# joaobuibergen/roms-trunk-mgh

Hardware: AMD Instinct MI355X
Metric: simulated-days/wall-sec (higher is better)
Workload: dtype f64; 1 GPU; BENCHMARK3 2048x256x30 NT=2 nonlinear 3-D step incl. 59 step2d calls, U3/C4 tracer advection, analytic atmospheric forcing, bulk fluxes + KPP + diagnostics every step; tiling=1x1, halo_transport=none, rccl_ranks=0, graph_exchanges=1, ndtfast=20, finite=True

## Files before the change

### include/roms_hip.h

```cpp
#ifndef ROMS_HIP_H
#define ROMS_HIP_H

#ifdef __cplusplus
extern "C" {
#endif

enum roms_kind {
  K_2D = 0, K_2D_T2, K_2D_T3, K_2D_NT,
  K_3DR, K_3DW, K_3DR_T2, K_3DW_T2, K_3DW_NAT, K_4DT, K_3DR_NT, K_3DW_T3
};

enum roms_field_id {
#define ROMS_FIELD(name, kind, owner) FID_##name,
#include "roms_fields.def"
#undef ROMS_FIELD
  FID_COUNT
};

typedef struct roms_fields {
#define ROMS_FIELD(name, kind, owner) double *name;
#include "roms_fields.def"
#undef ROMS_FIELD
} roms_fields_t;

// ... 129 lines not shown
int roms_hip_get_diagnostic(int dia_id, int itrc, int accumulated, double *host, long n_doubles);
int roms_hip_dia_index(int dia_id, int hdif, int rotated);
int roms_hip_set_floats(int Nfloats, const int *Ftype, const double *Tinfo, const double *Fz0,
                        const double *xcoord, const double *ycoord);
int roms_hip_floats_put(const double *track, long n_track, const int *bounded, long n_bounded);
int roms_hip_floats_get(double *track, long n_track, int *bounded, long n_bounded);
int roms_hip_step_floats(const roms_step_idx_t *s, double time, const int nfl[5]);
int roms_hip_set_tides(int NTC, int MTC, const double *Tperiod, const double *SSH_Tamp, const double *SSH_Tphase,
                       const double *UV_Tangle, const double *UV_Tphase, const double *UV_Tmajor, const double *UV_Tminor,
                       const double *angler, double tide_start, int ramp_tides, double dstart,
                       int add_fsobc, const double *zeta_base, int add_m2obc, const double *ubar_base,
                       const double *vbar_base);
int roms_hip_tides(double time);
int roms_hip_wvelocity(const roms_step_idx_t *s);
int roms_hip_diag(const roms_step_idx_t *s, double *out12);

int roms_hip_step2d_loop(roms_step_idx_t *s, int *indx1);

int roms_hip_graph_exchanges(int on);
int roms_hip_graph_exchanges_state(void);

int roms_hip_exchange(int field_id, int level);

typedef struct { int peer; int tag; long count; double *buf; } roms_halo_msg_t;
typedef int (*roms_halo_relay_fn)(void *user, int nsend, const roms_halo_msg_t *send,
                                  int nrecv, const roms_halo_msg_t *recv);
int roms_hip_set_halo_relay(roms_halo_relay_fn fn, void *user);
int roms_hip_halo_plan(const roms_bounds_t *b, int rank, int *out);

int roms_hip_timing_enable(int on);
// ... 11 lines not shown
```

### roms_trunk_mgh_amd/abi.py

```python
import ctypes as C
import keyword
import os
import re

ROOT = os.path.dirname(os.path.dirname(os.path.abspath(__file__)))
INCLUDE_DIR = os.path.join(ROOT, "include")


def _read(name):
    with open(os.path.join(INCLUDE_DIR, name)) as fh:
        return re.sub(r"/\*.*?\*/", "", fh.read(), flags=re.S)


def _constants():
    txt = _read("roms_hip.h")
    out = {n: int(v) for n, v in re.findall(r"^#define\s+(\w+)\s+(\d+)\s*$", txt, flags=re.M)}
    for body in re.findall(r"\benum\s+\w+\s*\{([^{}#]*)\}", txt):
        nxt = 0
        for item in body.split(","):
            name, _, val = (x.strip() for x in item.partition("="))
            out[name] = nxt = int(val) if val else nxt
            nxt += 1
    return out

# ... 7 lines not shown

ADV = {"C2": 0, "C4": 1, "A4": 2, "U3": 3, "SU3": 4, "SPLINES": 5,
       "MPDATA": 6, "HSIMT": 7}
GLS_STAB = {"GALPERIN": 0, "KANTHA_CLAYSON": 1, "CANUTO_A": 2, "CANUTO_B": 3}
PGF = {"DJ_GRADPS": 0, "STANDARD": 1, "WJ_GRADP": 2, "PJ_GRADP": 3}
LBC_PERIODIC, LBC_CLOSED, LBC_GRADIENT, LBC_CLAMPED, LBC_CHAPMAN_IMPLICIT, LBC_FLATHER, LBC_RADIATION = range(7)
LBC = {"Per": 0, "Clo": 1, "Gra": 2, "Cla": 3, "Cha": 4, "Fla": 5, "Rad": 6, "RadNud": 7, "Che": 8, "Shc": 9, "Red": 10}
UV_HADV = {"U3": 0, "C2": 1, "C4": 2}
UV_VADV = {"C4W": 0, "C2": 1, "C4": 2, "SPLINES": 3}
UV_ADV_PAIRS = [("U3", "C4W"), ("U3", "SPLINES"), ("C2", "C2"), ("C2", "SPLINES"), ("C4", "C4"), ("C4", "SPLINES")]


def uv_adv(h="U3", v="C4W"):
    return 1 | (UV_HADV.get(h, h) << 4) | (UV_VADV.get(v, v) << 8)


LBV = {"zeta": 0, "ubar": 1, "vbar": 2, "u": 3, "v": 4, "t": 5}
LBS = {"west": 0, "east": 1, "south": 2, "north": 3}


FIELDS = re.findall(r"\bROMS_FIELD\(\s*(\w+)\s*,\s*(\w+)\s*,\s*(\w+)\s*\)", _read("roms_fields.def"))
FIELD_ID = {n: i for i, (n, _, _) in enumerate(FIELDS)}
FIELD_KIND = {n: k for n, k, _ in FIELDS}


def trailing_shape(kind, N, NT, NAT):
    return {
        "K_2D": (), "K_2D_T2": (2,), "K_2D_T3": (3,), "K_2D_NT": (NT,),
        "K_3DR": (N,), "K_3DW": (N + 1,), "K_3DR_T2": (N, 2),
        "K_3DW_T2": (N + 1, 2), "K_3DW_NAT": (N + 1, NAT), "K_4DT": (N, 3, NT), "K_3DR_NT": (N, NT),
# ... 71 lines not shown
```

### roms_trunk_mgh_amd/csrc/capi.hip

```cpp
#include "roms_dev.h"
#include <algorithm>
#include <map>
#include <vector>

RomsCtx g_ctx;

static const int k_field_kind[FID_COUNT] = {
#define ROMS_FIELD(name, kind, owner) kind,
#include "roms_fields.def"
#undef ROMS_FIELD
};
static const char *k_field_name[FID_COUNT] = {
#define ROMS_FIELD(name, kind, owner) #name,
#include "roms_fields.def"
#undef ROMS_FIELD
};

int roms_fail(const char *where, const char *what)
{
  g_ctx.last_error = std::string(where) + ": " + what;
  return 8;
}

long roms_field_count(int kind, const roms_bounds_t &b)
// ... 23 lines not shown
  if (!g_ctx.timing) return;
  if (hipEventCreate(&e0) != hipSuccess || hipEventCreate(&e1) != hipSuccess) { e0 = e1 = nullptr; return; }
  (void)hipEventRecord(e0, g_ctx.stream);
}
ScopedTimer::~ScopedTimer()
{
  if (!e0) return;
  float ms = 0.f;
  if (hipEventRecord(e1, g_ctx.stream) == hipSuccess && hipEventSynchronize(e1) == hipSuccess &&
      hipEventElapsedTime(&ms, e0, e1) == hipSuccess)
    g_last_ms[name] = ms;
  (void)hipEventDestroy(e0);
  (void)hipEventDestroy(e1);
}

extern "C" int roms_hip_timing_enable(int on) { g_ctx.timing = on != 0; return 0; }
extern "C" double roms_hip_timing_last_ms(const char *entry)
{
  auto it = g_last_ms.find(entry);
  return it == g_last_ms.end() ? -1.0 : it->second;
}

__global__ void __launch_bounds__(256) k_calib_stream(const double *__restrict__ src, double *__restrict__ dst, long n)
{
  const long e = (long)blockIdx.x * 256 + threadIdx.x;
  if (e < n) dst[e] = src[e];
}
int roms_entry_check(const char *where);
namespace { void sources_release(); void clima_release(); void avg_release(); }
extern "C" int roms_hip_calib_stream(long n)
// ... 718 lines not shown
```

### roms_trunk_mgh_amd/csrc/k_diag.hip

```cpp
#include "roms_dev.h"

int roms_entry_check(const char *name);

namespace {

__global__ void __launch_bounds__(BLK_X *BLK_Y)
k_wvelocity(const RomsDev *__restrict__ c, int ninp)
{
  DEV_PROLOGUE(c)
  const Blk XB = xcd_block();
  const int i = b.Istr + XB.x * BLK_X + threadIdx.x;
  const int j = b.Jstr + XB.y * BLK_Y + threadIdx.y;
  if (i > b.Iend || j > b.Jend) return;
  const long a = I2(i, j);
  const gcd_t u = (gcd_t)(c->F.u + (long)(ninp - 1) * n3r), v = (gcd_t)(c->F.v + (long)(ninp - 1) * n3r);
  const gcd_t z_r = (gcd_t)c->F.z_r, z_w = (gcd_t)c->F.z_w, W = (gcd_t)c->F.W;
  const gd_t wvel = (gd_t)c->F.wvel;
  const gcd_t pm = (gcd_t)c->F.pm, pn = (gcd_t)c->F.pn;
  const double pmw = pm[a - 1] + pm[a], pme = pm[a] + pm[a + 1];
  const double pns = pn[a - ni] + pn[a], pnn = pn[a] + pn[a + ni];
  const double pmn = pm[a] * pn[a];
  auto vert_at = [&](int k) {
    const long q = a + (long)(k - 1) * nij;
    const double zr0 = z_r[q];
// ... 17 lines not shown
  }
  double vm = v1, v0 = v2, vp = v3;
  for (int k = 2; k <= N - 2; k++) {
    const double vq = vert_at(k + 2);
    wvel[w3i(k)] = pmn * (W[w3i(k)] + wrk * (z_w[w3i(k)] - zw0)) + cff4 * (v0 + vp) - cff5 * (vm + vq);
    vm = v0; v0 = vp; vp = vq;
  }
  {
    const long qN = a + (long)(N - 1) * nij;
    const double slope = (zwN - z_r[qN]) / (z_r[qN] - z_r[qN - nij]);
    wvel[w3i(N)] = pmn * wrk * (zwN - zw0) + cff1 * (vp + slope * (vp - v0)) + cff2 * vp - cff3 * v0;
    wvel[w3i(N - 1)] = pmn * (W[w3i(N - 1)] + wrk * (z_w[w3i(N - 1)] - zw0)) + cff1 * vp + cff2 * v0 - cff3 * vm;
  }
}

struct DiagScratch { double *ke, *pe, *C, *Cu, *Cv, *Cw, *Ck, *spd, *rho, *vol; };

__global__ void __launch_bounds__(BLK_X *BLK_Y)
k_diag_col(const RomsDev *__restrict__ c, int idia, DiagScratch w)
{
  DEV_PROLOGUE(c)
  const roms_params_t &p = c->p;
  const Blk XB = xcd_block();
  const int i = b.Istr + XB.x * BLK_X + threadIdx.x;
  const int j = b.Jstr + XB.y * BLK_Y + threadIdx.y;
  if (i > b.Iend || j > b.Jend) return;
  const long a = I2(i, j);
  const gcd_t u = (gcd_t)(c->F.u + (long)(idia - 1) * n3r), v = (gcd_t)(c->F.v + (long)(idia - 1) * n3r);
  const gcd_t Hz = (gcd_t)c->F.Hz, z_r = (gcd_t)c->F.z_r, z_w = (gcd_t)c->F.z_w, rho = (gcd_t)c->F.rho;
  const gcd_t wvel = (gcd_t)c->F.wvel;
  const double zwN = z_w[a + (long)N * nij], zw0 = z_w[a];
  const double pm = GF(pm)[a], pn = GF(pn)[a], dt = p.dt;
  double ke = 0.0, pe = 0.5 * p.g * zwN * zwN;
  const double cff = p.g / p.rho0;
  double mC = 0.0, mCu = 0.0, mCv = 0.0, mCw = 0.0, mspd = 0.0, mrho = -1.0E+37;
  int mk = 0;
  double wv_up = wvel[a + (long)N * nij];
  for (int k = N; k >= 1; k--) {
    const long q = a + (long)(k - 1) * nij;
    const double u0 = u[q], u1 = u[q + 1], v0 = v[q], v1 = v[q + ni], hz = Hz[q], rh = rho[q];
    const double wv_dn = wvel[q];
    const double u2v2 = u0 * u0 + u1 * u1 + v0 * v0 + v1 * v1;
    ke = ke + hz * 0.25 * u2v2;
    pe = pe + cff * hz * (rh + 1000.0) * (z_r[q] - zw0);
    const double Cu = 0.5 * fabs(u0 + u1) * dt * pm;
    const double Cv = 0.5 * fabs(v0 + v1) * dt * pn;
    const double Cw = 0.5 * fabs(wv_dn + wv_up) * dt / hz;
    const double C = Cu + Cv + Cw;
    if (C > mC) { mC = C; mCu = Cu; mCv = Cv; mCw = Cw; mk = k; }
    mspd = fmax(mspd, sqrt(0.5 * u2v2));
    mrho = fmax(mrho, rh);
    wv_up = wv_dn;
  }
  const double om = GF(omn)[a];
  w.vol[a] = om * (zwN - zw0);
  ke = om * ke;
  pe = om * pe;
  w.ke[a] = ke; w.pe[a] = pe; w.C[a] = mC; w.Cu[a] = mCu; w.Cv[a] = mCv; w.Cw[a] = mCw; w.Ck[a] = (double)mk;
  w.spd[a] = mspd; w.rho[a] = mrho;
}

enum { R_VOL = 0, R_PE, R_KE, R_C, R_CU, R_CV, R_CW, R_CJ, R_CK, R_SPD, R_RHO, R_COUNT };

#define DIAG_UNR 16
__global__ void __launch_bounds__(64)
k_diag_rows(const RomsDev *__restrict__ c, DiagScratch w, double *__restrict__ R)
{
  DEV_PROLOGUE(c)
  const int i = b.Istr + blockIdx.x * blockDim.x + threadIdx.x;
  if (i > b.Iend) return;
  const int nI = b.Iend - b.Istr + 1, o = i - b.Istr;
  const gcd_t gvol = (gcd_t)w.vol, gpe = (gcd_t)w.pe, gke = (gcd_t)w.ke, gC = (gcd_t)w.C, gspd = (gcd_t)w.spd,
              grho = (gcd_t)w.rho;
  double vol = 0.0, pe = 0.0, ke = 0.0, mC = 0.0, mCu = 0.0, mCv = 0.0, mCw = 0.0, mspd = 0.0, mrho = -1.0E+37;
// ... 136 lines not shown
  const roms_bounds_t &b = g_ctx.b;
  if (b.N < 3) return roms_fail("roms_hip_wvelocity", "needs N >= 3");
  halo_batch_begin();
  halo_exchange2d(GT_U, g_ctx.dev[FID_DU_avg1]);
  halo_exchange2d(GT_V, g_ctx.dev[FID_DV_avg1]);
  if ((rc = halo_batch_end())) return rc;
  {
    ScopedTimer tm("wvelocity");
    hipLaunchKernelGGL(k_wvelocity, grid2d(b.Iend - b.Istr + 1, b.Jend - b.Jstr + 1), block2d(), 0, g_ctx.stream,
                       g_ctx.devc, s->nstp);
    KERNEL_CHECK("k_wvelocity");
  }
  return bc_w3d(g_ctx.dev[FID_wvel]);
}

extern "C" int roms_hip_diag(const roms_step_idx_t *s, double *out12)
{
  int rc = roms_entry_check("roms_hip_diag");
  if (rc) return rc;
  if (!out12) return roms_fail("roms_hip_diag", "null output");
  const roms_bounds_t &b = g_ctx.b;
  const int nI = b.Iend - b.Istr + 1, nJ = b.Jend - b.Jstr + 1;
  if (!g_diag_dev) HIP_TRY(hipMalloc(&g_diag_dev, 12 * sizeof(double)));
  if (g_diag_rows_n < (long)R_COUNT * nI) {
    if (g_diag_rows) HIP_TRY(hipFree(g_diag_rows));
    g_diag_rows = nullptr;
    HIP_TRY(hipMalloc(&g_diag_rows, sizeof(double) * R_COUNT * nI));
    g_diag_rows_n = (long)R_COUNT * nI;
  }
  double **ws = g_ctx.hostc.ws2;
  DiagScratch w{ws[8], ws[9], ws[10], ws[11], ws[12], ws[13], ws[14], ws[15], ws[16], ws[17]};
  {
    ScopedTimer tm("diag");
    hipLaunchKernelGGL(k_diag_col, grid2d(nI, nJ), block2d(), 0, g_ctx.stream, g_ctx.devc, s->nstp, w);
    KERNEL_CHECK("k_diag_col");
    hipLaunchKernelGGL(k_diag_rows, dim3((nI + 63) / 64), dim3(64), 0, g_ctx.stream, g_ctx.devc, w, g_diag_rows);
    KERNEL_CHECK("k_diag_rows");
    hipLaunchKernelGGL(k_diag_final, dim3(1), dim3(256), 0, g_ctx.stream, g_ctx.devc, (const double *)g_diag_rows,
                       g_diag_dev);
    KERNEL_CHECK("k_diag_final");
  }
  HIP_TRY(hipMemcpyAsync(out12, g_diag_dev, 12 * sizeof(double), hipMemcpyDeviceToHost, g_ctx.stream));
  HIP_TRY(hipStreamSynchronize(g_ctx.stream));
  return 0;
}
```

### roms_trunk_mgh_amd/csrc/k_rho_eos.hip

```cpp
#include "roms_dev.h"
#include "roms_eoscoef.h"

int roms_entry_check(const char *name);

namespace {

struct EosPt {
  double den1, bulk0, bulk1, bulk2, bulk, den;
  double Dden1DS, Dden1DT, DbulkDS, DbulkDT;
};

template <bool DERIV>
__device__ __forceinline__ EosPt eos_point(double tt, double ts, double Tp)
{
  EosPt o;
  const double Tt = (-2.0 > tt) ? -2.0 : tt;
  const double Ts = (0.0 > ts) ? 0.0 : ts;
  const double sqrtTs = sqrt(Ts);
  const double Tpr10 = 0.1 * Tp;
  const double C0 = EOS_Q00 + Tt * (EOS_Q01 + Tt * (EOS_Q02 + Tt * (EOS_Q03 + Tt * (EOS_Q04 + Tt * EOS_Q05))));
  const double C1 = EOS_U00 + Tt * (EOS_U01 + Tt * (EOS_U02 + Tt * (EOS_U03 + Tt * EOS_U04)));
  const double C2 = EOS_V00 + Tt * (EOS_V01 + Tt * EOS_V02);
  o.den1 = C0 + Ts * (C1 + sqrtTs * C2 + Ts * EOS_W00);
  const double C3 = EOS_A00 + Tt * (EOS_A01 + Tt * (EOS_A02 + Tt * (EOS_A03 + Tt * EOS_A04)));
// ... 17 lines not shown
    o.Dden1DS = C1 + 1.5 * C2 * sqrtTs + 2.0 * EOS_W00 * Ts;
    o.Dden1DT = d0 + Ts * (d1 + sqrtTs * d2);
    const double d3 = EOS_A01 + Tt * (2.0 * EOS_A02 + Tt * (3.0 * EOS_A03 + Tt * 4.0 * EOS_A04));
    const double d4 = EOS_B01 + Tt * (2.0 * EOS_B02 + Tt * 3.0 * EOS_B03);
    const double d5 = EOS_D01 + Tt * 2.0 * EOS_D02;
    const double d6 = EOS_E01 + Tt * (2.0 * EOS_E02 + Tt * 3.0 * EOS_E03);
    const double d7 = EOS_F01 + Tt * 2.0 * EOS_F02;
    const double d8 = EOS_G02 + Tt * 2.0 * EOS_G03;
    const double d9 = EOS_H01 + Tt * 2.0 * EOS_H02;
    o.DbulkDS = C4 + sqrtTs * 1.5 * C5 - Tp * (C7 + sqrtTs * 1.5 * EOS_G00 - Tp * C9);
    o.DbulkDT = d3 + Ts * (d4 + sqrtTs * d5) - Tp * (d6 + Ts * d7 - Tp * (d8 + Ts * d9));
  }
  return o;
}

__global__ void __launch_bounds__(BLK_X *BLK_Y)
k_rho_eos_nonlin(const RomsDev *__restrict__ c, int nrhs)
{
  DEV_PROLOGUE(c)
  const Blk XB = xcd_block();
  const int i = b.IstrT + XB.x * BLK_X + threadIdx.x;
  const int j = b.JstrT + XB.y * BLK_Y + threadIdx.y;
  if (i > b.IendT || j > b.JendT) return;
  const long c0 = I2(i, j);
  const gcd_t T = (gcd_t)(c->F.t + (long)(nrhs - 1) * n3r);
  const gcd_t S = (gcd_t)(c->F.t + ((long)(nrhs - 1) + 3L) * n3r);
  const bool salt = c->p.salinity != 0 && b.NT >= 2;
  const gcd_t z_r = (gcd_t)(c->F.z_r);
  const gcd_t z_w = (gcd_t)(c->F.z_w);
  const gcd_t Hz = (gcd_t)(c->F.Hz);
  const double g = c->p.g;
  double rhoA = 0.0, rhoS = 0.0;
  EosPt up{};
  double zr_up = 0.0;
  const bool masking = c->p.masking != 0;
  const double rm = masking ? GF(rmask)[c0] : 1.0;
  for (int k = N; k >= 1; k--) {
    const long ck = c0 + (long)(k - 1) * nij;
    const double zr = z_r[ck], hz = Hz[ck];
    const double tt = T[ck], ts = salt ? S[ck] : 0.0;
    EosPt e;
    if (k == N) {
      e = eos_point<true>(tt, ts, zr);
      if (masking) e.den = e.den * rm;
      const double Tpr10 = 0.1 * zr;
      const double cff = e.bulk + Tpr10;
      const double cff1 = Tpr10 * e.den1;
      const double cff2 = e.bulk * cff;
      const double wrk = (e.den + 1000.0) * cff * cff;
      const double Tcof = -(e.DbulkDT * cff1 + e.Dden1DT * cff2);
      const double Scof = (e.DbulkDS * cff1 + e.Dden1DS * cff2);
// ... 9 lines not shown
      if (masking) e.den = e.den * rm;
      const double cf1 = e.den * hz;
      rhoS = rhoS + hz * (rhoA + 0.5 * cf1);
      rhoA = rhoA + cf1;
      const double zw = z_w[c0 + (long)k * nij];
      const double bulk_up = up.bulk0 - zw * (up.bulk1 - up.bulk2 * zw);
      const double bulk_dn = e.bulk0 - zw * (e.bulk1 - e.bulk2 * zw);
      const double c1 = 1.0 / (bulk_up + 0.1 * zw);
      const double c2 = 1.0 / (bulk_dn + 0.1 * zw);
      const double den_up = c1 * (up.den1 * bulk_up);
      const double den_dn = c2 * (e.den1 * bulk_dn);
      GF(bvf)[c0 + (long)k * nij] = -g * (den_up - den_dn) / (0.5 * (den_up + den_dn) * (zr_up - zr));
    }
    GF(rho)[ck] = e.den;
    GF(pden)[ck] = masking ? (e.den1 - 1000.0) * rm : e.den1 - 1000.0;
    up = e;
    zr_up = zr;
  }
  GF(bvf)[c0] = 0.0;
  const double cff2 = 1.0 / c->p.rho0;
  const double cff1 = 1.0 / (z_w[c0 + (long)N * nij] - z_w[c0]);
  GF(rhoA)[c0] = cff2 * cff1 * rhoA;
  GF(rhoS)[c0] = 2.0 * cff1 * cff1 * cff2 * rhoS;
}

__global__ void __launch_bounds__(BLK_X *BLK_Y)
k_rho_eos_lin(const RomsDev *__restrict__ c, int nrhs)
{
  DEV_PROLOGUE(c)
  const Blk XB = xcd_block();
  const int i = b.IstrT + XB.x * BLK_X + threadIdx.x;
  const int j = b.JstrT + XB.y * BLK_Y + threadIdx.y;
  if (i > b.IendT || j > b.JendT) return;
  const long c0 = I2(i, j);
  const gcd_t T = (gcd_t)(c->F.t + (long)(nrhs - 1) * n3r);
  const gcd_t S = (gcd_t)(c->F.t + ((long)(nrhs - 1) + 3L) * n3r);
  const bool salt = c->p.salinity != 0 && b.NT >= 2;
  const double R0 = c->p.R0, T0 = c->p.T0, S0 = c->p.S0, Tcoef = c->p.Tcoef, Scoef = c->p.Scoef;
// ... 11 lines not shown
    if (k == N) { rhoS = 0.5 * cf1 * hz; rhoA = cf1; }
    else { rhoS = rhoS + hz * (rhoA + 0.5 * cf1); rhoA = rhoA + cf1; }
  }
  const double cff2 = 1.0 / c->p.rho0;
  const double cff1 = 1.0 / (GF(z_w)[c0 + (long)N * nij] - GF(z_w)[c0]);
  GF(rhoA)[c0] = cff2 * cff1 * rhoA;
  GF(rhoS)[c0] = 2.0 * cff1 * cff1 * cff2 * rhoS;
}

}

extern "C" int roms_hip_rho_eos(const roms_step_idx_t *s)
{
  int rc = roms_entry_check("roms_hip_rho_eos");
  if (rc) return rc;
  ScopedTimer tm("rho_eos");
  const roms_bounds_t &b = g_ctx.b;
  dim3 grid = grid2d(b.IendT - b.IstrT + 1, b.JendT - b.JstrT + 1);
  if (g_ctx.p.nonlin_eos)
    hipLaunchKernelGGL(k_rho_eos_nonlin, grid, block2d(), 0, g_ctx.stream, g_ctx.devc, s->nrhs);
  else
    hipLaunchKernelGGL(k_rho_eos_lin, grid, block2d(), 0, g_ctx.stream, g_ctx.devc, s->nrhs);
  KERNEL_CHECK("k_rho_eos");
  halo_batch_begin();
  halo_exchange3d(GT_R, b.N, g_ctx.dev[FID_rho]);
  halo_exchange3d(GT_R, b.N, g_ctx.dev[FID_pden]);
  halo_exchange2d(GT_R, g_ctx.dev[FID_rhoA]);
  halo_exchange2d(GT_R, g_ctx.dev[FID_rhoS]);
  if (g_ctx.p.nonlin_eos) {
    halo_exchange2d(GT_R, g_ctx.dev[FID_alpha]);
    halo_exchange2d(GT_R, g_ctx.dev[FID_beta]);
    halo_exchange3d(GT_R, b.N + 1, g_ctx.dev[FID_bvf]);
  }
  return halo_batch_end();
}
// ... 1 lines not shown
```

### roms_trunk_mgh_amd/hip.py

```python
import ctypes as C
import os

import numpy as np

from . import abi

_HERE = os.path.dirname(os.path.abspath(__file__))
LIB_PATH = os.path.join(_HERE, "libroms_hip.so")
_LIB = None


def use_library(path):
    global LIB_PATH
    if _LIB is not None:
        raise RuntimeError("use_library() after the library was loaded")
    LIB_PATH = os.path.abspath(path)

ENTRIES = ["set_massflux", "rho_eos", "omega", "set_zeta", "set_depth", "rhs3d",
           "pre_step3d", "prsgrd", "t3dmix2", "rhs3d_tile", "uv3dmix2", "step2d",
           "step3d_uv", "step3d_t", "bulk_flux", "set_vbc", "lmd_vmix", "wvelocity", "ini_zeta", "ini_fields",
           "t3dmix4", "uv3dmix4", "gls_prestep", "gls_corstep", "wetdry", "set_avg", "set_diags"]

DECLARED_SYMBOLS = (
    ["roms_hip_init", "roms_hip_finalize", "roms_hip_get_unique_id", "roms_hip_set_bounds",
     "roms_hip_set_params", "roms_hip_register_field", "roms_hip_sync_to_device",
     "roms_hip_sync_to_host", "roms_hip_sync_all_to_device", "roms_hip_sync_all_to_host",
     "roms_hip_device_ptr", "roms_hip_device_synchronize", "roms_hip_last_error",
     "roms_hip_step2d_loop", "roms_hip_exchange", "roms_hip_timing_enable",
     "roms_hip_timing_last_ms", "roms_hip_calib_stream", "roms_hip_set_halo_relay", "roms_hip_diag",
     "roms_hip_snapshot_begin", "roms_hip_snapshot_end", "roms_hip_halo_plan",
     "roms_hip_ana_srflux", "roms_hip_check_guards", "roms_hip_row_metrics_state",
     "roms_hip_graph_exchanges", "roms_hip_graph_exchanges_state", "roms_hip_set_sources",
     "roms_hip_set_clima", "roms_hip_set_averages", "roms_hip_get_average", "roms_hip_average_device_ptr",
     "roms_hip_avg_phase", "roms_hip_set_floats", "roms_hip_floats_put", "roms_hip_floats_get",
     "roms_hip_step_floats", "roms_hip_set_tides", "roms_hip_tides", "roms_hip_set_diagnostics",
     "roms_hip_get_diagnostic", "roms_hip_dia_index"] + ["roms_hip_" + e for e in ENTRIES])


_DP = C.POINTER(C.c_double)
class HaloMsg(C.Structure):
    _fields_ = [("peer", C.c_int), ("tag", C.c_int), ("count", C.c_long), ("buf", _DP)]


RELAY_FN = C.CFUNCTYPE(C.c_int, C.c_void_p, C.c_int, C.POINTER(HaloMsg), C.c_int, C.POINTER(HaloMsg))


def load():
    global _LIB
    if _LIB is not None:
        return _LIB
    if not os.path.exists(LIB_PATH):
# ... 27 lines not shown
    lib.roms_hip_get_average.argtypes = [C.c_int, C.c_int, C.c_void_p, C.c_long]
    lib.roms_hip_average_device_ptr.restype = C.c_void_p
    lib.roms_hip_average_device_ptr.argtypes = [C.c_int, C.c_int]
    lib.roms_hip_avg_phase.argtypes = [C.c_int] * 5
    lib.roms_hip_set_floats.argtypes = [C.c_int, _ip, _DP, _DP, _DP, _DP]
    lib.roms_hip_floats_put.argtypes = [C.c_void_p, C.c_long, C.c_void_p, C.c_long]
    lib.roms_hip_floats_get.argtypes = [C.c_void_p, C.c_long, C.c_void_p, C.c_long]
    lib.roms_hip_step_floats.argtypes = [C.POINTER(abi.StepIdx), C.c_double, _ip]
    lib.roms_hip_set_tides.argtypes = ([C.c_int, C.c_int] + [_DP] * 8 + [C.c_double, C.c_int, C.c_double, C.c_int, _DP,
                                        C.c_int, _DP, _DP])
    lib.roms_hip_tides.argtypes = [C.c_double]
    lib.roms_hip_set_diagnostics.argtypes = [C.c_int] * 4
    lib.roms_hip_get_diagnostic.argtypes = [C.c_int, C.c_int, C.c_int, C.c_void_p, C.c_long]
    lib.roms_hip_dia_index.argtypes = [C.c_int] * 3
    lib.roms_hip_set_halo_relay.argtypes = [RELAY_FN, C.c_void_p]
    if hasattr(lib, "roms_hip_tile_neighbors"):
        lib.roms_hip_tile_neighbors.argtypes = [C.c_int] * 7 + [C.POINTER(C.c_int)]
    _LIB = lib
    return lib


def tile_neighbors(rank, ntileI, ntileJ, Nghost, NghostPoints, EWperiodic, NSperiodic):
    out = (C.c_int * 12)()
    load().roms_hip_tile_neighbors(rank, ntileI, ntileJ, Nghost, NghostPoints,
                                   int(EWperiodic), int(NSperiodic), out)
    keys = ["Wtile", "Etile", "Stile", "Ntile", "GsendW", "GsendE", "GrecvW", "GrecvE",
            "GsendS", "GsendN", "GrecvS", "GrecvN"]
    return dict(zip(keys, list(out)))


# ... 127 lines not shown

    def snapshot_end(self):
        self._chk(self.l.roms_hip_snapshot_end(), "snapshot_end")

    def ana_srflux(self, yday, hour):
        self.l.roms_hip_ana_srflux.argtypes = [C.c_double, C.c_double]
        self._chk(self.l.roms_hip_ana_srflux(float(yday), float(hour)), "ana_srflux")

    def diag(self, s):
        import numpy as np
        out = np.zeros(12)
        self.l.roms_hip_diag.argtypes = [C.POINTER(abi.StepIdx), _DP]
        self._chk(self.l.roms_hip_diag(C.byref(s), out.ctypes.data_as(_DP)), "diag")
        return out

    def step2d_loop(self, s, indx1):
        ii = C.c_int(indx1)
        self._chk(self.l.roms_hip_step2d_loop(C.byref(s), C.byref(ii)), "step2d_loop")
        return ii.value

    def to_device(self, names=None):
        if names is None:
            self._chk(self.l.roms_hip_sync_all_to_device(), "sync_all_to_device")
        else:
            for n in names:
                self._chk(self.l.roms_hip_sync_to_device(abi.FIELD_ID[n]), "sync_to_device")

    def to_host(self, names=None):
        if names is None:
            self._chk(self.l.roms_hip_sync_all_to_host(), "sync_all_to_host")
# ... 72 lines not shown
```

### roms_trunk_mgh_amd/main3d.py

```python
from . import abi


def host_clock(tdays):
    import math
    dn = 367.0 + tdays
    frac = abs(dn - math.trunc(dn))
    day = math.trunc(dn) - 367
    if not 0 <= day < 365:
        raise ValueError("host_clock covers the first 365 days only")
    return float(day + 1) + frac, round(frac * 86400.0) / 3600.0


class Main3D:
    def __init__(self, backend, ntstart=1, physics=False, diagnostics=False, ninfo=1, averages=None, floats=None, tides=None,
                 diags=None):
        self.be = backend
        self.tides = tides
        if tides is not None:
            backend.set_tides(tides)
        self.floats = floats
        if floats is not None:
            backend.set_floats(floats)
        self.diags = diags
        if diags is not None:
            backend.set_diagnostics(diags)
        self.averages = averages
        if averages is not None:
            backend.set_averages(averages)
        self.physics = physics
        self.diagnostics = diagnostics
        self.ninfo = ninfo
        self.last_diag = None
        self.iic = ntstart
        self.ntstart = ntstart
        self.ntfirst = ntstart
        self.indx1 = 1
        self.s = abi.StepIdx(iic=ntstart, ntfirst=ntstart, nstp=1, nnew=2, nrhs=1,
                             kstp=1, krhs=1, knew=1, iif=1, predictor_2d_step=0)

    def initial(self):
        s = self.s
        s.nstp, s.nnew, s.nrhs = 1, 2, 1
        if self.be.st.p.wet_dry:
            s.kstp = 1
            self.be.call("wetdry", s)
        for k in ("set_depth", "set_massflux", "omega", "rho_eos"):
            self.be.call(k, s)

    def _rotate(self):
        s = self.s
        s.iic = self.iic
        s.ntfirst = self.ntfirst
        s.nstp = 1 + (self.iic - self.ntstart) % 2
        s.nnew = 3 - s.nstp
        s.nrhs = s.nstp

    def step(self):
        be, s = self.be, self
        self._rotate()
        s = self.s
        if self.iic == self.ntstart:
            be.call("ini_zeta", s)
            be.call("set_depth", s)
            be.call("ini_fields", s)
        be.call("set_massflux", s)
        be.call("rho_eos", s)
        if self.diagnostics and (self.iic - 1) % self.ninfo == 0:
            self.last_diag = be.diag(s)
        bench_app = getattr(be.st, "cfg", {}).get("app") == "BENCHMARK"
        if self.physics:
            if bench_app:
                dt = be.st.p.dt
                be.ana_srflux(*host_clock((self.iic - self.ntstart) * dt / 86400.0))
            if bench_app:
                be.call("bulk_flux", s)
            be.call("set_vbc", s)
        if self.tides is not None:
            be.tides((self.iic - self.ntstart) * be.st.p.dt)
        if self.physics and bench_app:
            be.call("lmd_vmix", s)
        be.call("omega", s)
        if self.diagnostics:
            be.call("wvelocity", s)
        be.call("set_zeta", s)
        if self.diags is not None:
            be.call("set_diags", s)
        if self.averages is not None:
            be.call("set_avg", s)
        be.call("rhs3d", s)
        gls = bool(be.st.p.gls_mixing)
        if gls:
            be.call("gls_prestep", s)
        self.indx1 = be.step2d_loop(s, self.indx1)
        be.call("set_depth", s)
        be.call("step3d_uv", s)
        be.call("omega", s)
        if gls:
            be.call("gls_corstep", s)
# ... 20 lines not shown
```

Measured before the change: 0.2407 simulated-days/s.

## Fuse step-front kernels: massflux+omega+wvelocity and diag into rho_eos

Adds a step_front entry that runs the start of each 3-D step through one C call. Set_massflux, omega and wvelocity are computed by a single column kernel that keeps the vertical integral in registers. The diagnostic column pass is folded into the nonlinear rho_eos kernel. This cuts kernel launches, Python-to-C calls and repeated reads of Hz, u, v and z_r, at the cost of a large register-heavy templated kernel and duplicated logic that must stay in sync with the separate entries.

```diff
diff --git a/include/roms_hip.h b/include/roms_hip.h
--- a/include/roms_hip.h
+++ b/include/roms_hip.h
@@ -167,6 +167,9 @@
 int roms_hip_tides(double time);
 int roms_hip_wvelocity(const roms_step_idx_t *s);
 int roms_hip_diag(const roms_step_idx_t *s, double *out12);
+enum roms_front_flag { ROMS_FRONT_SRFLUX = 1, ROMS_FRONT_BULK = 2, ROMS_FRONT_VBC = 4, ROMS_FRONT_LMD = 8,
+                       ROMS_FRONT_DIAG = 16, ROMS_FRONT_WVEL = 32 };
+int roms_hip_step_front(const roms_step_idx_t *s, int flags, double yday, double hour, double *diag12);
 
 int roms_hip_step2d_loop(roms_step_idx_t *s, int *indx1);
 
diff --git a/roms_trunk_mgh_amd/abi.py b/roms_trunk_mgh_amd/abi.py
--- a/roms_trunk_mgh_amd/abi.py
+++ b/roms_trunk_mgh_amd/abi.py
@@ -45,6 +45,8 @@
 def uv_adv(h="U3", v="C4W"):
     return 1 | (UV_HADV.get(h, h) << 4) | (UV_VADV.get(v, v) << 8)
 
+
+FRONT = {n: CONSTANTS["ROMS_FRONT_" + n] for n in ("SRFLUX", "BULK", "VBC", "LMD", "DIAG", "WVEL")}
 
 LBV = {"zeta": 0, "ubar": 1, "vbar": 2, "u": 3, "v": 4, "t": 5}
 LBS = {"west": 0, "east": 1, "south": 2, "north": 3}
diff --git a/roms_trunk_mgh_amd/csrc/capi.hip b/roms_trunk_mgh_amd/csrc/capi.hip
--- a/roms_trunk_mgh_amd/csrc/capi.hip
+++ b/roms_trunk_mgh_amd/csrc/capi.hip
@@ -61,6 +61,7 @@
   (void)hipEventDestroy(e1);
 }
 
+void timing_forget(const char *name) { g_last_ms.erase(name); }
 extern "C" int roms_hip_timing_enable(int on) { g_ctx.timing = on != 0; return 0; }
 extern "C" double roms_hip_timing_last_ms(const char *entry)
 {
diff --git a/roms_trunk_mgh_amd/csrc/diag.h b/roms_trunk_mgh_amd/csrc/diag.h
--- /dev/null
+++ b/roms_trunk_mgh_amd/csrc/diag.h
@@ -0,0 +1,47 @@
+#pragma once
+#include "roms_dev.h"
+
+struct DiagScratch { double *ke, *pe, *C, *Cu, *Cv, *Cw, *Ck, *spd, *rho, *vol; };
+
+#ifdef __HIPCC__
+struct DiagCol {
+  double ke, pe, mC, mCu, mCv, mCw, mspd, mrho, wv_up;
+  int mk;
+  __device__ __forceinline__ void begin(double g, double zwN, double wvN)
+  {
+    ke = 0.0; pe = 0.5 * g * zwN * zwN;
+    mC = 0.0; mCu = 0.0; mCv = 0.0; mCw = 0.0; mspd = 0.0; mrho = -1.0E+37;
+    mk = 0;
+    wv_up = wvN;
+  }
+  __device__ __forceinline__ void level(int k, double u0, double u1, double v0, double v1, double hz, double rh, double dz,
+                                        double wv_dn, double cff, double dt, double pm, double pn)
+  {
+    const double u2v2 = u0 * u0 + u1 * u1 + v0 * v0 + v1 * v1;
+    ke = ke + hz * 0.25 * u2v2;
+    pe = pe + cff * hz * (rh + 1000.0) * dz;
+    const double Cu = 0.5 * fabs(u0 + u1) * dt * pm;
+    const double Cv = 0.5 * fabs(v0 + v1) * dt * pn;
+    const double Cw = 0.5 * fabs(wv_dn + wv_up) * dt / hz;
+    const double C = Cu + Cv + Cw;
+    if (C > mC) { mC = C; mCu = Cu; mCv = Cv; mCw = Cw; mk = k; }
+    mspd = fmax(mspd, sqrt(0.5 * u2v2));
+    mrho = fmax(mrho, rh);
+    wv_up = wv_dn;
+  }
+  __device__ __forceinline__ void store(const DiagScratch &w, long a, double om, double zwN, double zw0)
+  {
+    w.vol[a] = om * (zwN - zw0);
+    ke = om * ke;
+    pe = om * pe;
+    w.ke[a] = ke; w.pe[a] = pe; w.C[a] = mC; w.Cu[a] = mCu; w.Cv[a] = mCv; w.Cw[a] = mCw; w.Ck[a] = (double)mk;
+    w.spd[a] = mspd; w.rho[a] = mrho;
+  }
+};
+#endif
+
+int diag_prepare(DiagScratch *w);
+int diag_reduce();
+int diag_fetch(double *out12);
+int rho_eos_entry(const roms_step_idx_t *s, const DiagScratch *w, int idia);
+void timing_forget(const char *name);
diff --git a/roms_trunk_mgh_amd/csrc/k_diag.hip b/roms_trunk_mgh_amd/csrc/k_diag.hip
--- a/roms_trunk_mgh_amd/csrc/k_diag.hip
+++ b/roms_trunk_mgh_amd/csrc/k_diag.hip
@@ -1,4 +1,5 @@
 #include "roms_dev.h"
+#include "diag.h"
 
 int roms_entry_check(const char *name);
 
@@ -55,8 +56,6 @@
   }
 }
 
-struct DiagScratch { double *ke, *pe, *C, *Cu, *Cv, *Cw, *Ck, *spd, *rho, *vol; };
-
 __global__ void __launch_bounds__(BLK_X *BLK_Y)
 k_diag_col(const RomsDev *__restrict__ c, int idia, DiagScratch w)
 {
@@ -72,33 +71,14 @@
   const gcd_t wvel = (gcd_t)c->F.wvel;
   const double zwN = z_w[a + (long)N * nij], zw0 = z_w[a];
   const double pm = GF(pm)[a], pn = GF(pn)[a], dt = p.dt;
-  double ke = 0.0, pe = 0.5 * p.g * zwN * zwN;
   const double cff = p.g / p.rho0;
-  double mC = 0.0, mCu = 0.0, mCv = 0.0, mCw = 0.0, mspd = 0.0, mrho = -1.0E+37;
-  int mk = 0;
-  double wv_up = wvel[a + (long)N * nij];
+  DiagCol d;
+  d.begin(p.g, zwN, wvel[a + (long)N * nij]);
   for (int k = N; k >= 1; k--) {
     const long q = a + (long)(k - 1) * nij;
-    const double u0 = u[q], u1 = u[q + 1], v0 = v[q], v1 = v[q + ni], hz = Hz[q], rh = rho[q];
-    const double wv_dn = wvel[q];
-    const double u2v2 = u0 * u0 + u1 * u1 + v0 * v0 + v1 * v1;
-    ke = ke + hz * 0.25 * u2v2;
-    pe = pe + cff * hz * (rh + 1000.0) * (z_r[q] - zw0);
-    const double Cu = 0.5 * fabs(u0 + u1) * dt * pm;
-    const double Cv = 0.5 * fabs(v0 + v1) * dt * pn;
-    const double Cw = 0.5 * fabs(wv_dn + wv_up) * dt / hz;
-    const double C = Cu + Cv + Cw;
-    if (C > mC) { mC = C; mCu = Cu; mCv = Cv; mCw = Cw; mk = k; }
-    mspd = fmax(mspd, sqrt(0.5 * u2v2));
-    mrho = fmax(mrho, rh);
-    wv_up = wv_dn;
-  }
-  const double om = GF(omn)[a];
-  w.vol[a] = om * (zwN - zw0);
-  ke = om * ke;
-  pe = om * pe;
-  w.ke[a] = ke; w.pe[a] = pe; w.C[a] = mC; w.Cu[a] = mCu; w.Cv[a] = mCv; w.Cw[a] = mCw; w.Ck[a] = (double)mk;
-  w.spd[a] = mspd; w.rho[a] = mrho;
+    d.level(k, u[q], u[q + 1], v[q], v[q + ni], Hz[q], rho[q], z_r[q] - zw0, wvel[q], cff, dt, pm, pn);
+  }
+  d.store(w, a, GF(omn)[a], zwN, zw0);
 }
 
 enum { R_VOL = 0, R_PE, R_KE, R_C, R_CU, R_CV, R_CW, R_CJ, R_CK, R_SPD, R_RHO, R_COUNT };
@@ -265,13 +245,9 @@
   return bc_w3d(g_ctx.dev[FID_wvel]);
 }
 
-extern "C" int roms_hip_diag(const roms_step_idx_t *s, double *out12)
-{
-  int rc = roms_entry_check("roms_hip_diag");
-  if (rc) return rc;
-  if (!out12) return roms_fail("roms_hip_diag", "null output");
-  const roms_bounds_t &b = g_ctx.b;
-  const int nI = b.Iend - b.Istr + 1, nJ = b.Jend - b.Jstr + 1;
+int diag_prepare(DiagScratch *w)
+{
+  const int nI = g_ctx.b.Iend - g_ctx.b.Istr + 1;
   if (!g_diag_dev) HIP_TRY(hipMalloc(&g_diag_dev, 12 * sizeof(double)));
   if (g_diag_rows_n < (long)R_COUNT * nI) {
     if (g_diag_rows) HIP_TRY(hipFree(g_diag_rows));
@@ -280,18 +256,45 @@
     g_diag_rows_n = (long)R_COUNT * nI;
   }
   double **ws = g_ctx.hostc.ws2;
-  DiagScratch w{ws[8], ws[9], ws[10], ws[11], ws[12], ws[13], ws[14], ws[15], ws[16], ws[17]};
+  *w = DiagScratch{ws[8], ws[9], ws[10], ws[11], ws[12], ws[13], ws[14], ws[15], ws[16], ws[17]};
+  return 0;
+}
+
+int diag_reduce()
+{
+  DiagScratch w;
+  int rc = diag_prepare(&w);
+  if (rc) return rc;
+  const int nI = g_ctx.b.Iend - g_ctx.b.Istr + 1;
+  hipLaunchKernelGGL(k_diag_rows, dim3((nI + 63) / 64), dim3(64), 0, g_ctx.stream, g_ctx.devc, w, g_diag_rows);
+  KERNEL_CHECK("k_diag_rows");
+  hipLaunchKernelGGL(k_diag_final, dim3(1), dim3(256), 0, g_ctx.stream, g_ctx.devc, (const double *)g_diag_rows,
+                     g_diag_dev);
+  KERNEL_CHECK("k_diag_final");
+  return 0;
+}
+
+int diag_fetch(double *out12)
+{
+  HIP_TRY(hipMemcpyAsync(out12, g_diag_dev, 12 * sizeof(double), hipMemcpyDeviceToHost, g_ctx.stream));
+  HIP_TRY(hipStreamSynchronize(g_ctx.stream));
+  return 0;
+}
+
+extern "C" int roms_hip_diag(const roms_step_idx_t *s, double *out12)
+{
+  int rc = roms_entry_check("roms_hip_diag");
+  if (rc) return rc;
+  if (!out12) return roms_fail("roms_hip_diag", "null output");
+  const roms_bounds_t &b = g_ctx.b;
+  const int nI = b.Iend - b.Istr + 1, nJ = b.Jend - b.Jstr + 1;
+  DiagScratch w;
+  if ((rc = diag_prepare(&w))) return rc;
   {
     ScopedTimer tm("diag");
     hipLaunchKernelGGL(k_diag_col, grid2d(nI, nJ), block2d(), 0, g_ctx.stream, g_ctx.devc, s->nstp, w);
     KERNEL_CHECK("k_diag_col");
-    hipLaunchKernelGGL(k_diag_rows, dim3((nI + 63) / 64), dim3(64), 0, g_ctx.stream, g_ctx.devc, w, g_diag_rows);
-    KERNEL_CHECK("k_diag_rows");
-    hipLaunchKernelGGL(k_diag_final, dim3(1), dim3(256), 0, g_ctx.stream, g_ctx.devc, (const double *)g_diag_rows,
-                       g_diag_dev);
-    KERNEL_CHECK("k_diag_final");
-  }
-  HIP_TRY(hipMemcpyAsync(out12, g_diag_dev, 12 * sizeof(double), hipMemcpyDeviceToHost, g_ctx.stream));
-  HIP_TRY(hipStreamSynchronize(g_ctx.stream));
-  return 0;
-}
+    if ((rc = diag_reduce())) return rc;
+  }
+  return diag_fetch(out12);
+}
diff --git a/roms_trunk_mgh_amd/csrc/k_front.hip b/roms_trunk_mgh_amd/csrc/k_front.hip
--- /dev/null
+++ b/roms_trunk_mgh_amd/csrc/k_front.hip
@@ -0,0 +1,184 @@
+#include "roms_dev.h"
+#include "diag.h"
+
+int roms_entry_check(const char *name);
+
+namespace {
+
+template <int NMAX, bool WVEL>
+__global__ void __launch_bounds__(BLK_X *BLK_Y)
+k_front_flux(const RomsDev *__restrict__ c, int nrhs)
+{
+  DEV_PROLOGUE(c)
+  const Blk XB = xcd_block();
+  const int i = b.IstrT + XB.x * BLK_X + threadIdx.x;
+  const int j = b.JstrT + XB.y * BLK_Y + threadIdx.y;
+  if (i > b.IendT || j > b.JendT) return;
+  const long a = I2(i, j);
+  const gcd_t Hz = (gcd_t)(c->F.Hz);
+  const gcd_t u = (gcd_t)(c->F.u + (long)(nrhs - 1) * n3r);
+  const gcd_t v = (gcd_t)(c->F.v + (long)(nrhs - 1) * n3r);
+  const gd_t Huon = (gd_t)(c->F.Huon), Hvom = (gd_t)(c->F.Hvom);
+  if (i < b.Istr || i > b.Iend || j < b.Jstr || j > b.Jend) {
+    const bool su = i >= b.IstrP, sv = j >= b.JstrP;
+    const double on_u = GF(on_u)[a], om_v = GF(om_v)[a];
+    for (int k = 1; k <= N; k++) {
+      const long q = a + (long)(k - 1) * nij;
+      const double hz = Hz[q];
+      if (su) Huon[q] = 0.5 * (hz + Hz[q - 1]) * u[q] * on_u;
+      if (sv) Hvom[q] = 0.5 * (hz + Hz[q - ni]) * v[q] * om_v;
+    }
+    return;
+  }
+  const gcd_t z_r = (gcd_t)c->F.z_r, z_w = (gcd_t)c->F.z_w;
+  const double on_u0 = GF(on_u)[a], on_u1 = GF(on_u)[a + 1], om_v0 = GF(om_v)[a], om_v1 = GF(om_v)[a + ni];
+  double pmw = 0.0, pme = 0.0, pns = 0.0, pnn = 0.0;
+  if constexpr (WVEL) {
+    const gcd_t pm = (gcd_t)c->F.pm, pn = (gcd_t)c->F.pn;
+    pmw = pm[a - 1] + pm[a]; pme = pm[a] + pm[a + 1];
+    pns = pn[a - ni] + pn[a]; pnn = pn[a] + pn[a + ni];
+  }
+  double w[NMAX + 1];
+  double vert[WVEL ? NMAX + 1 : 1];
+  double zr1 = 0.0, zr2 = 0.0, zrN = 0.0, zrN1 = 0.0;
+  w[0] = 0.0;
+#pragma unroll
+  for (int k = 1; k <= NMAX; k++) {
+    if (k <= N) {
+      const long q = a + (long)(k - 1) * nij;
+      const double hz = Hz[q], u0 = u[q], u1 = u[q + 1], v0 = v[q], v1 = v[q + ni];
+      const double hu0 = 0.5 * (hz + Hz[q - 1]) * u0 * on_u0;
+      const double hu1 = 0.5 * (Hz[q + 1] + hz) * u1 * on_u1;
+      const double hv0 = 0.5 * (hz + Hz[q - ni]) * v0 * om_v0;
+      const double hv1 = 0.5 * (Hz[q + ni] + hz) * v1 * om_v1;
+      Huon[q] = hu0;
+      Hvom[q] = hv0;
+      w[k] = w[k - 1] - (hu1 - hu0 + hv1 - hv0);
+      if constexpr (WVEL) {
+        const double zr0 = z_r[q];
+        const double wu0 = u0 * (zr0 - z_r[q - 1]) * pmw;
+        const double wu1 = u1 * (z_r[q + 1] - zr0) * pme;
+        double ve = 0.25 * (wu0 + wu1);
+        const double wv0 = v0 * (zr0 - z_r[q - ni]) * pns;
+        const double wv1 = v1 * (z_r[q + ni] - zr0) * pnn;
+        ve = ve + 0.25 * (wv0 + wv1);
+        vert[k] = ve;
+        if (k == 1) zr1 = zr0;
+        if (k == 2) zr2 = zr0;
+        if (k == N - 1) zrN1 = zr0;
+        if (k == N) zrN = zr0;
+      }
+    } else if constexpr (WVEL) {
+      vert[k] = 0.0;
+    }
+  }
+  const double zw0 = z_w[a], zwN = z_w[a + (long)N * nij];
+  double wN = 0.0;
+#pragma unroll
+  for (int k = 1; k <= NMAX; k++) if (k == N) wN = w[k];
+  const double wrkW = wN / (zwN - zw0);
+  const gd_t W = (gd_t)(c->F.W);
+  const gd_t wvel = (gd_t)c->F.wvel;
+  const double cff1 = 3.0 / 8.0, cff2 = 3.0 / 4.0, cff3 = 1.0 / 8.0, cff4 = 9.0 / 16.0, cff5 = 1.0 / 16.0;
+  double wrk = 0.0, pmn = 0.0;
+  W[a] = 0.0;
+  if constexpr (WVEL) {
+    wrk = (GF(DU_avg1)[a] - GF(DU_avg1)[a + 1] + GF(DV_avg1)[a] - GF(DV_avg1)[a + ni]) / (zwN - zw0);
+    pmn = GF(pm)[a] * GF(pn)[a];
+    const double slope = (zr1 - zw0) / (zr2 - zr1);
+    wvel[a] = cff1 * (vert[1] - slope * (vert[2] - vert[1])) + cff2 * vert[1] - cff3 * vert[2];
+  }
+#pragma unroll
+  for (int k = 1; k < NMAX; k++) {
+    if (k < N) {
+      const long qw = a + (long)k * nij;
+      const double zw = z_w[qw];
+      const double Wk = w[k] - wrkW * (zw - zw0);
+      W[qw] = Wk;
+      if constexpr (WVEL) {
+        const double vm = vert[k > 1 ? k - 1 : 1], v0 = vert[k], vp = vert[k + 1], vq = vert[k + 2 <= NMAX ? k + 2 : NMAX];
+        double x;
+        if (k == N - 1) x = pmn * (Wk + wrk * (zw - zw0)) + cff1 * vp + cff2 * v0 - cff3 * vm;
+        else if (k == 1) x = pmn * (Wk + wrk * (zw - zw0)) + cff1 * v0 + cff2 * vp - cff3 * vq;
+        else x = pmn * (Wk + wrk * (zw - zw0)) + cff4 * (v0 + vp) - cff5 * (vm + vq);
+        wvel[qw] = x;
+      }
+    }
+  }
+  W[a + (long)N * nij] = 0.0;
+  if constexpr (WVEL) {
+    double vN = 0.0, vN1 = 0.0;
+#pragma unroll
+    for (int k = 2; k <= NMAX; k++) if (k == N) { vN = vert[k]; vN1 = vert[k - 1]; }
+    const double slope = (zwN - zrN) / (zrN - zrN1);
+    wvel[a + (long)N * nij] = pmn * wrk * (zwN - zw0) + cff1 * (vN + slope * (vN - vN1)) + cff2 * vN - cff3 * vN1;
+  }
+}
+
+template <bool WVEL>
+void launch_front_flux(const roms_step_idx_t *s)
+{
+  const roms_bounds_t &b = g_ctx.b;
+  const dim3 grid = grid2d(b.IendT - b.IstrT + 1, b.JendT - b.JstrT + 1);
+  if (b.N <= 16) hipLaunchKernelGGL((k_front_flux<16, WVEL>), grid, block2d(), 0, g_ctx.stream, g_ctx.devc, s->nrhs);
+  else if (b.N <= 32) hipLaunchKernelGGL((k_front_flux<32, WVEL>), grid, block2d(), 0, g_ctx.stream, g_ctx.devc, s->nrhs);
+  else hipLaunchKernelGGL((k_front_flux<ROMS_MAXN, WVEL>), grid, block2d(), 0, g_ctx.stream, g_ctx.devc, s->nrhs);
+}
+
+}
+
+extern "C" int roms_hip_step_front(const roms_step_idx_t *s, int flags, double yday, double hour, double *diag12)
+{
+  const char *me = "roms_hip_step_front";
+  int rc = roms_entry_check(me);
+  if (rc) return rc;
+  if ((rc = check_lbc())) return rc;
+  const roms_bounds_t &b = g_ctx.b;
+  const bool diag = (flags & ROMS_FRONT_DIAG) != 0, wvel = (flags & ROMS_FRONT_WVEL) != 0;
+  if (flags & ~(ROMS_FRONT_SRFLUX | ROMS_FRONT_BULK | ROMS_FRONT_VBC | ROMS_FRONT_LMD | ROMS_FRONT_DIAG | ROMS_FRONT_WVEL))
+    return roms_fail(me, "unknown flag");
+  if (diag && !diag12) return roms_fail(me, "ROMS_FRONT_DIAG without an output vector");
+  if (wvel && b.N < 3) return roms_fail(me, "wvelocity needs N >= 3");
+  if (s->nrhs != s->nstp) return roms_fail(me, "nrhs = nstp at the front of the step (main3d.F:189-191)");
+  if (g_ctx.p.point_sources & 3)
+    return roms_fail(me, "point sources are not covered: run the separate entries");
+  if (g_ctx.p.gls_mixing) return roms_fail(me, "GLS / MY25 mixing is not covered: run the separate entries");
+
+  const bool fused_diag = diag && g_ctx.p.nonlin_eos;
+  DiagScratch w;
+  if (diag && (rc = diag_prepare(&w))) return rc;
+  if ((rc = rho_eos_entry(s, fused_diag ? &w : nullptr, s->nstp))) return rc;
+  if (fused_diag) {
+    ScopedTimer tm("diag");
+    if ((rc = diag_reduce())) return rc;
+  } else if (diag) {
+    if ((rc = roms_hip_diag(s, diag12))) return rc;
+  }
+  if ((flags & ROMS_FRONT_SRFLUX) && (rc = roms_hip_ana_srflux(yday, hour))) return rc;
+  if ((flags & ROMS_FRONT_BULK) && (rc = roms_hip_bulk_flux(s))) return rc;
+  if ((flags & ROMS_FRONT_VBC) && (rc = roms_hip_set_vbc(s))) return rc;
+  if ((flags & ROMS_FRONT_LMD) && (rc = roms_hip_lmd_vmix(s))) return rc;
+  if (wvel) {
+    halo_batch_begin();
+    halo_exchange2d(GT_U, g_ctx.dev[FID_DU_avg1]);
+    halo_exchange2d(GT_V, g_ctx.dev[FID_DV_avg1]);
+    if ((rc = halo_batch_end())) return rc;
+  }
+  {
+    ScopedTimer tm("set_massflux");
+    if (wvel) launch_front_flux<true>(s);
+    else launch_front_flux<false>(s);
+    KERNEL_CHECK("k_front_flux");
+  }
+  if (g_ctx.timing) {
+    if (wvel) timing_forget("wvelocity");
+  }
+  halo_batch_begin();
+  halo_exchange3d(GT_U, b.N, g_ctx.dev[FID_Huon]);
+  halo_exchange3d(GT_V, b.N, g_ctx.dev[FID_Hvom]);
+  if ((rc = halo_batch_end())) return rc;
+  if ((rc = bc_w3d(g_ctx.dev[FID_W]))) return rc;
+  if (wvel && (rc = bc_w3d(g_ctx.dev[FID_wvel]))) return rc;
+  if (fused_diag) return diag_fetch(diag12);
+  return 0;
+}
diff --git a/roms_trunk_mgh_amd/csrc/k_rho_eos.hip b/roms_trunk_mgh_amd/csrc/k_rho_eos.hip
--- a/roms_trunk_mgh_amd/csrc/k_rho_eos.hip
+++ b/roms_trunk_mgh_amd/csrc/k_rho_eos.hip
@@ -1,4 +1,5 @@
 #include "roms_dev.h"
+#include "diag.h"
 #include "roms_eoscoef.h"
 
 int roms_entry_check(const char *name);
@@ -55,8 +56,9 @@
   return o;
 }
 
+template <bool DIAG>
 __global__ void __launch_bounds__(BLK_X *BLK_Y)
-k_rho_eos_nonlin(const RomsDev *__restrict__ c, int nrhs)
+k_rho_eos_nonlin(const RomsDev *__restrict__ c, int nrhs, int idia, DiagScratch dw)
 {
   DEV_PROLOGUE(c)
   const Blk XB = xcd_block();
@@ -76,6 +78,17 @@
   double zr_up = 0.0;
   const bool masking = c->p.masking != 0;
   const double rm = masking ? GF(rmask)[c0] : 1.0;
+  const bool dg = DIAG && i >= b.Istr && i <= b.Iend && j >= b.Jstr && j <= b.Jend;
+  const gcd_t du = (gcd_t)(c->F.u + (long)(idia - 1) * n3r), dv = (gcd_t)(c->F.v + (long)(idia - 1) * n3r);
+  const gcd_t wvel = (gcd_t)c->F.wvel;
+  DiagCol d;
+  double d_zw0 = 0.0, d_zwN = 0.0, d_pm = 0.0, d_pn = 0.0;
+  const double d_cff = g / c->p.rho0, d_dt = c->p.dt;
+  if (dg) {
+    d_zw0 = z_w[c0]; d_zwN = z_w[c0 + (long)N * nij];
+    d_pm = GF(pm)[c0]; d_pn = GF(pn)[c0];
+    d.begin(g, d_zwN, wvel[c0 + (long)N * nij]);
+  }
   for (int k = N; k >= 1; k--) {
     const long ck = c0 + (long)(k - 1) * nij;
     const double zr = z_r[ck], hz = Hz[ck];
@@ -115,6 +128,7 @@
     }
     GF(rho)[ck] = e.den;
     GF(pden)[ck] = masking ? (e.den1 - 1000.0) * rm : e.den1 - 1000.0;
+    if (dg) d.level(k, du[ck], du[ck + 1], dv[ck], dv[ck + ni], hz, e.den, zr - d_zw0, wvel[ck], d_cff, d_dt, d_pm, d_pn);
     up = e;
     zr_up = zr;
   }
@@ -123,6 +137,7 @@
   const double cff1 = 1.0 / (z_w[c0 + (long)N * nij] - z_w[c0]);
   GF(rhoA)[c0] = cff2 * cff1 * rhoA;
   GF(rhoS)[c0] = 2.0 * cff1 * cff1 * cff2 * rhoS;
+  if (dg) d.store(dw, c0, GF(omn)[c0], d_zwN, d_zw0);
 }
 
 __global__ void __launch_bounds__(BLK_X *BLK_Y)
@@ -164,11 +179,19 @@
 {
   int rc = roms_entry_check("roms_hip_rho_eos");
   if (rc) return rc;
+  return rho_eos_entry(s, nullptr, 0);
+}
+
+int rho_eos_entry(const roms_step_idx_t *s, const DiagScratch *w, int idia)
+{
+  if (w && !g_ctx.p.nonlin_eos) return roms_fail("rho_eos_entry", "the linear equation of state has no diag instantiation");
   ScopedTimer tm("rho_eos");
   const roms_bounds_t &b = g_ctx.b;
   dim3 grid = grid2d(b.IendT - b.IstrT + 1, b.JendT - b.JstrT + 1);
-  if (g_ctx.p.nonlin_eos)
-    hipLaunchKernelGGL(k_rho_eos_nonlin, grid, block2d(), 0, g_ctx.stream, g_ctx.devc, s->nrhs);
+  if (w)
+    hipLaunchKernelGGL(k_rho_eos_nonlin<true>, grid, block2d(), 0, g_ctx.stream, g_ctx.devc, s->nrhs, idia, *w);
+  else if (g_ctx.p.nonlin_eos)
+    hipLaunchKernelGGL(k_rho_eos_nonlin<false>, grid, block2d(), 0, g_ctx.stream, g_ctx.devc, s->nrhs, 1, DiagScratch{});
   else
     hipLaunchKernelGGL(k_rho_eos_lin, grid, block2d(), 0, g_ctx.stream, g_ctx.devc, s->nrhs);
   KERNEL_CHECK("k_rho_eos");
diff --git a/roms_trunk_mgh_amd/hip.py b/roms_trunk_mgh_amd/hip.py
--- a/roms_trunk_mgh_amd/hip.py
+++ b/roms_trunk_mgh_amd/hip.py
@@ -34,7 +34,7 @@
      "roms_hip_set_clima", "roms_hip_set_averages", "roms_hip_get_average", "roms_hip_average_device_ptr",
      "roms_hip_avg_phase", "roms_hip_set_floats", "roms_hip_floats_put", "roms_hip_floats_get",
      "roms_hip_step_floats", "roms_hip_set_tides", "roms_hip_tides", "roms_hip_set_diagnostics",
-     "roms_hip_get_diagnostic", "roms_hip_dia_index"] + ["roms_hip_" + e for e in ENTRIES])
+     "roms_hip_get_diagnostic", "roms_hip_dia_index", "roms_hip_step_front"] + ["roms_hip_" + e for e in ENTRIES])
 
 
 _DP = C.POINTER(C.c_double)
@@ -92,6 +92,7 @@
     lib.roms_hip_get_diagnostic.argtypes = [C.c_int, C.c_int, C.c_int, C.c_void_p, C.c_long]
     lib.roms_hip_dia_index.argtypes = [C.c_int] * 3
     lib.roms_hip_set_halo_relay.argtypes = [RELAY_FN, C.c_void_p]
+    lib.roms_hip_step_front.argtypes = [C.POINTER(abi.StepIdx), C.c_int, C.c_double, C.c_double, _DP]
     if hasattr(lib, "roms_hip_tile_neighbors"):
         lib.roms_hip_tile_neighbors.argtypes = [C.c_int] * 7 + [C.POINTER(C.c_int)]
     _LIB = lib
@@ -249,6 +250,12 @@
         self._chk(self.l.roms_hip_diag(C.byref(s), out.ctypes.data_as(_DP)), "diag")
         return out
 
+    def step_front(self, s, flags, yday=0.0, hour=0.0):
+        out = np.zeros(12)
+        self._chk(self.l.roms_hip_step_front(C.byref(s), int(flags), float(yday), float(hour), out.ctypes.data_as(_DP)),
+                  "step_front")
+        return out if flags & abi.FRONT["DIAG"] else None
+
     def step2d_loop(self, s, indx1):
         ii = C.c_int(indx1)
         self._chk(self.l.roms_hip_step2d_loop(C.byref(s), C.byref(ii)), "step2d_loop")
diff --git a/roms_trunk_mgh_amd/main3d.py b/roms_trunk_mgh_amd/main3d.py
--- a/roms_trunk_mgh_amd/main3d.py
+++ b/roms_trunk_mgh_amd/main3d.py
@@ -13,7 +13,7 @@
 
 class Main3D:
     def __init__(self, backend, ntstart=1, physics=False, diagnostics=False, ninfo=1, averages=None, floats=None, tides=None,
-                 diags=None):
+                 diags=None, front=True):
         self.be = backend
         self.tides = tides
         if tides is not None:
@@ -30,6 +30,7 @@
         self.physics = physics
         self.diagnostics = diagnostics
         self.ninfo = ninfo
+        self.front = front
         self.last_diag = None
         self.iic = ntstart
         self.ntstart = ntstart
@@ -55,6 +56,22 @@
         s.nnew = 3 - s.nstp
         s.nrhs = s.nstp
 
+    def _front_flags(self, bench_app):
+        be = self.be
+        if not self.front or not hasattr(be, "step_front") or "diag" in vars(be):
+            return None
+        if self.tides is not None or self.diags is not None or self.averages is not None:
+            return None
+        if be.st.p.gls_mixing or (be.st.p.point_sources & 3):
+            return None
+        F = abi.FRONT
+        flags = 0
+        if self.physics:
+            flags |= F["VBC"] | ((F["SRFLUX"] | F["BULK"] | F["LMD"]) if bench_app else 0)
+        if self.diagnostics:
+            flags |= F["WVEL"] | (F["DIAG"] if (self.iic - 1) % self.ninfo == 0 else 0)
+        return flags
+
     def step(self):
         be, s = self.be, self
         self._rotate()
@@ -63,11 +80,23 @@
             be.call("ini_zeta", s)
             be.call("set_depth", s)
             be.call("ini_fields", s)
+        bench_app = getattr(be.st, "cfg", {}).get("app") == "BENCHMARK"
+        flags = self._front_flags(bench_app)
+        if flags is None:
+            self._front_calls(bench_app)
+        else:
+            clock = host_clock((self.iic - self.ntstart) * be.st.p.dt / 86400.0) if flags & abi.FRONT["SRFLUX"] else (0.0, 0.0)
+            d = be.step_front(s, flags, *clock)
+            if d is not None:
+                self.last_diag = d
+        self._rest_of_step()
+
+    def _front_calls(self, bench_app):
+        be, s = self.be, self.s
         be.call("set_massflux", s)
         be.call("rho_eos", s)
         if self.diagnostics and (self.iic - 1) % self.ninfo == 0:
             self.last_diag = be.diag(s)
-        bench_app = getattr(be.st, "cfg", {}).get("app") == "BENCHMARK"
         if self.physics:
             if bench_app:
                 dt = be.st.p.dt
@@ -82,6 +111,9 @@
         be.call("omega", s)
         if self.diagnostics:
             be.call("wvelocity", s)
+
+    def _rest_of_step(self):
+        be, s = self.be, self.s
         be.call("set_zeta", s)
         if self.diags is not None:
             be.call("set_diags", s)
```

After: 0.2435 simulated-days/s, median of 6. About the same (+1.2%).
